# JuliaParallel/DistributedArrays.jl

Measured on NVIDIA H100. Metric: GB/s for map! and sum on Float32 DArray, higher is better.
Workload: dtype f32

## Files before the change

### distributedarrays.jl_b200/_broadcast.py

```python
from __future__ import annotations

import ctypes as C
import struct
from typing import Callable, List, Optional, Sequence, Tuple

import numpy as np

from builtins import any as builtins_any

from . import _lib
from ._darray import B200Array, DArray, dab_dtype, darray, makelocal
from .layout import shape_of
from .runtime import close_remote_reads, open_remote_reads, runtime

_RANK = {"bool": 0, "i32": 1, "i64": 2, "i128": 3, "f32": 4, "f64": 5}


class _TagTypes(dict):

    def __missing__(self, tag):
        raise _lib.UnsupportedError(_lib.ERR_UNSUPPORTED, f"values of type {tag} have no array element type on the GPU backend "
                                    "(Int128 is served as the value type of mapreduce(f, op, d) only)")


# ... 310 lines not shown
        raise _lib.UnsupportedError(_lib.ERR_UNSUPPORTED, "cis of a complex value is not served (complex transcendental functions)")
    e = _float_of(e)
    return Expr("cis", (e,), _CPLX_OF[e.jt])


def complex_(x, y=None) -> Expr:
    e = _traced(x, "complex")
    if y is None:
        if is_ctag(e.jt):
            return e
        if e.jt not in _CPLX_OF:
            raise _lib.UnsupportedError(_lib.ERR_UNSUPPORTED, f"complex({e.jt}) would be Complex{{{e.jt}}}: only ComplexF32 / ComplexF64 are served")
        return convert(e, _CPLX_OF[e.jt])
    f = Expr.wrap(y)
    if is_ctag(e.jt) or is_ctag(f.jt):
        raise TypeError("MethodError: complex(x, y) takes two real parts")
    jt = promote(e.jt, f.jt)
    if jt not in _CPLX_OF:
        raise _lib.UnsupportedError(_lib.ERR_UNSUPPORTED, f"complex of {jt} parts would be Complex{{{jt}}}: only ComplexF32 / ComplexF64 are served")
    return Expr("complex", (convert(e, jt), convert(f, jt)), _CPLX_OF[jt])


def iszero(x) -> Expr:
    return binop("eq", _traced(x, "iszero"), Expr.wrap(0))


def _traced(x, name: str) -> Expr:
    if isinstance(x, Expr):
        return x
    raise TypeError(f"dab.{name} is for use inside broadcast/map kernels")


def uses_complex(e: Expr) -> bool:
    return is_ctag(e.jt) or builtins_any(uses_complex(a) for a in e.args)


def ifelse(c, a, b) -> Expr:
    c, a, b = Expr.wrap(c), Expr.wrap(a), Expr.wrap(b)
    jt = promote(a.jt, b.jt)
    return Expr("ifelse", (convert(c, "bool"), convert(a, jt), convert(b, jt)), jt)


def _mk_unary(name):
    def f(x):
        if isinstance(x, Expr):
            return unop(name, x)
        raise TypeError(f"dab.{name} is for use inside broadcast/map kernels")

    f.__name__ = name
    return f


abs2 = _mk_unary("abs2")
sqrt = _mk_unary("sqrt")
inv = _mk_unary("inv")
floor = _mk_unary("floor")
ceil = _mk_unary("ceil")
sign = _mk_unary("sign")
sin = _mk_unary("sin")
cos = _mk_unary("cos")
tan = _mk_unary("tan")
exp = _mk_unary("exp")
log = _mk_unary("log")
tanh = _mk_unary("tanh")
isnan = _mk_unary("isnan")
isinf = _mk_unary("isinf")
isfinite = _mk_unary("isfinite")
# ... 172 lines not shown
        groups.append((o, ext))
    if not groups:
        groups = [(1, [1] * len(shapes))]
    return tuple(g[0] for g in groups), [tuple(g[1][k] for g in groups) for k in range(len(shapes))]


def _dense_strides(shape):
    s, out = 1, []
    for d in shape:
        out.append(s)
        s *= int(d)
    return out


class LocalArg:

    def __init__(self, arr: Optional[B200Array] = None, scalar=None, tag: str = "f64", temp: bool = False):
        self.arr, self.scalar, self.tag, self.temp = arr, scalar, tag, temp


def run_local(rt, expr: Expr, out: B200Array, largs: List[LocalArg]):
    n = out.size
    if n == 0:
        return
    out_tag = tag_of(out.dtype)
    full = [a for a in largs if a.arr is not None]
    same = all(a.arr.shape == out.shape or a.arr.size == n and _squeeze(a.arr.shape) == _squeeze(out.shape) for a in full)
    ctx = rt.ctx
    code = dab_dtype(out.dtype)
    rt.last_kernel = "fixed"
    cplx = uses_complex(expr) or builtins_any(is_ctag(a.tag) for a in largs)
    if same and not cplx and expr.jt == out_tag and out_tag != "bool":
        x0 = largs[0] if largs and largs[0].arr is not None and largs[0].tag == out_tag else None
        if x0 is not None and all(_only_arg0(expr)):
            ab = match_affine(expr)
            if ab is not None:
                a = np.asarray(ab[0], dtype=out.dtype)
                b = np.asarray(ab[1], dtype=out.dtype)
                _lib.call("dab_affine", ctx, code, C.c_void_p(out.ptr), C.c_void_p(x0.arr.ptr), C.c_void_p(a.ctypes.data),
                          C.c_void_p(b.ctypes.data), n)
                rt.last_kernel = "dab_affine"
                return
            if expr.op in _UN and _is_arg(expr.args[0], 0):
                _lib.call("dab_unary", ctx, code, _UN[expr.op], C.c_void_p(out.ptr), C.c_void_p(x0.arr.ptr), n)
                return
            if _is_arg(expr, 0):
                _lib.call("dab_unary", ctx, code, _lib.MAP_ID, C.c_void_p(out.ptr), C.c_void_p(x0.arr.ptr), n)
                return
        if expr.op in _BIN and len(expr.args) == 2 and not (expr.op == "div" and out_tag[0] != "f"):
            l, r = expr.args
            la = largs[l.val] if l.op == "arg" else None
            ra = largs[r.val] if r.op == "arg" else None

            def arr_ok(e, a):
                return e.op == "arg" and a is not None and a.arr is not None and a.tag == out_tag

            def sc_val(e, a):
                if e.op == "const" and e.jt == out_tag:
                    return e.val
                if e.op == "arg" and a is not None and a.arr is None and a.tag == out_tag:
                    return a.scalar
                return None

            if arr_ok(l, la) and arr_ok(r, ra):
                _lib.call("dab_binary", ctx, code, _BIN[expr.op], C.c_void_p(out.ptr), C.c_void_p(la.arr.ptr), C.c_void_p(ra.arr.ptr), n)
                return
            if arr_ok(l, la) and sc_val(r, ra) is not None:
# ... 43 lines not shown
                    strides[4 * k + d] = 0
                else:
                    raise _lib.DimensionMismatch(_lib.ERR_DIM_MISMATCH, f"arrays could not be broadcast: {a.arr.shape} vs {out.shape}")
        else:
            ptrs[k] = None
            scal[k] = struct.unpack("<Q", np.asarray(a.scalar, dtype=_NPT[a.tag]).tobytes().ljust(8, b"\0"))[0]
    _lib.call("dab_broadcast_expr", ctx, src, code, C.c_void_p(out.ptr), _lib.sz4(oshape), _lib.sz4(_dense_strides(oshape)), nargs, dts,
              ptrs, strides, scal)


def split_c128_scalars(expr: Expr, largs: List["LocalArg"]):
    ks = [k for k, a in enumerate(largs) if a.arr is None and a.tag == "c128"]
    if not ks:
        return expr, largs
    largs, sub = list(largs), {}
    for k in ks:
        z = complex(largs[k].scalar)
        largs[k] = LocalArg(None, z.real, "f64")
        largs.append(LocalArg(None, z.imag, "f64"))
        sub[k] = Expr("complex", (Expr("arg", (), "f64", k), Expr("arg", (), "f64", len(largs) - 1)), "c128")

    def rw(e: Expr) -> Expr:
        if e.op == "arg":
            return sub.get(e.val, e)
        return Expr(e.op, tuple(rw(a) for a in e.args), e.jt, e.val, e.weak) if e.args else e

    return rw(expr), largs


def _squeeze(shape):
    return tuple(s for s in shape if s != 1)


def _only_arg0(e: Expr):
    if e.op == "arg":
        yield e.val == 0
    elif e.op != "const":
        for a in e.args:
            yield from _only_arg0(a)




def _bc_shape(shapes: Sequence[Tuple[int, ...]]) -> Tuple[int, ...]:
    nd = max((len(s) for s in shapes), default=0)
    out = []
    for k in range(nd):
        ext = 1
        for s in shapes:
            v = s[k] if k < len(s) else 1
            if v != 1:
                if ext != 1 and ext != v:
                    raise _lib.DimensionMismatch(_lib.ERR_DIM_MISMATCH, f"arrays could not be broadcast to a common size: {shapes}")
                ext = v
        out.append(ext)
    return tuple(out)


def _arg_tag(a) -> str:
    if isinstance(a, (DArray,)):
        return tag_of(a.dtype)
    if isinstance(a, np.ndarray) and a.ndim > 0:
        return tag_of(a.dtype)
    return Expr.wrap(a.item() if isinstance(a, np.ndarray) else a).jt


def _bcview(arg_dims: Sequence[int], I) -> Tuple:
    out = []
    for k, s in enumerate(arg_dims):
        if s == 1:
            out.append((1, 1))
        elif k < len(I):
# ... 163 lines not shown
```

### distributedarrays.jl_b200/_darray.py

```python
from __future__ import annotations

import ctypes as C
import itertools
import weakref
from typing import Callable, Dict, List, Optional, Sequence, Tuple

import numpy as np

from . import _lib
from .layout import Layout, Range, default_procs, layout_from_chunk_shapes, make_layout, rlen, shape_of, slab_plan
from .runtime import Runtime, close_remote_reads, open_remote_reads, runtime

_DT = {np.dtype(np.float32): _lib.F32, np.dtype(np.float64): _lib.F64, np.dtype(np.int32): _lib.I32,
       np.dtype(np.int64): _lib.I64, np.dtype(np.bool_): _lib.U8,
       np.dtype(np.complex64): _lib.C64, np.dtype(np.complex128): _lib.C128}
_NP = {_lib.F32: np.dtype(np.float32), _lib.F64: np.dtype(np.float64), _lib.I32: np.dtype(np.int32),
       _lib.I64: np.dtype(np.int64), _lib.U8: np.dtype(np.bool_), _lib.C64: np.dtype(np.complex64), _lib.C128: np.dtype(np.complex128)}


def dab_dtype(dt) -> int:
    dt = np.dtype(dt)
    if dt not in _DT:
        raise _lib.UnsupportedError(_lib.ERR_UNSUPPORTED, f"element type {dt} is not served by the GPU backend (no host fallback)")
    return _DT[dt]


def np_dtype(code: int) -> np.dtype:
    return _NP[code]


def is_complex(dt) -> bool:
    return np.dtype(dt).kind == "c"


def component_dtype(dt) -> np.dtype:
    dt = np.dtype(dt)
# ... 2 lines not shown

_allowscalar = [True]


def allowscalar(flag: bool = True):
    _allowscalar[0] = bool(flag)


class B200Array:

    __slots__ = ("rt", "ptr", "shape", "dtype", "_own", "_keep", "_temp")

    def __init__(self, rt: Runtime, ptr: int, shape: Sequence[int], dtype, own: bool = True, keep=None, temp: bool = False):
        self.rt, self.ptr, self.shape, self.dtype = rt, int(ptr), tuple(int(s) for s in shape), np.dtype(dtype)
        self._own, self._keep, self._temp = own, keep, temp

    @classmethod
    def empty(cls, rt: Runtime, shape: Sequence[int], dtype, temp: bool = False) -> "B200Array":
        dtype = np.dtype(dtype)
        n = int(np.prod(shape)) if len(shape) else 1
        ptr = rt.alloc_temp(n * dtype.itemsize) if temp else rt.alloc(n * dtype.itemsize)
        return cls(rt, ptr, shape, dtype, temp=temp)

    @classmethod
    def from_numpy(cls, rt: Runtime, a: np.ndarray) -> "B200Array":
        a = np.asarray(a)
        dab_dtype(a.dtype)
        out = cls.empty(rt, a.shape, a.dtype)
        out.copy_from_host(a)
        return out

    @property
    def size(self) -> int:
        return int(np.prod(self.shape)) if len(self.shape) else 1

    @property
    def nbytes(self) -> int:
        return self.size * self.dtype.itemsize

    @property
    def ndim(self) -> int:
        return len(self.shape)

    def copy_from_host(self, a: np.ndarray, sync: bool = True):
        a = np.asarray(a, dtype=self.dtype)
        if tuple(a.shape) != self.shape:
            raise _lib.DimensionMismatch(_lib.ERR_DIM_MISMATCH, f"host array {a.shape} vs chunk {self.shape}")
        if self.size == 0:
            return
        if not a.flags.f_contiguous:
            if a.ndim == 2 and a.strides[0] == a.itemsize and a.strides[1] > 0:
                _lib.call("dab_h2d_2d", self.rt.ctx, C.c_void_p(self.ptr), a.shape[0] * a.itemsize, C.c_void_p(a.ctypes.data),
                          a.strides[1], a.shape[0] * a.itemsize, a.shape[1])
                if sync:
                    self.rt.sync()
                return
            a = np.asfortranarray(a)
        _lib.call("dab_h2d", self.rt.ctx, C.c_void_p(self.ptr), C.c_void_p(a.ctypes.data), self.nbytes)
        if sync:
            self.rt.sync()

    def to_numpy(self) -> np.ndarray:
        out = np.empty(self.shape, dtype=self.dtype, order="F")
        if self.size:
            _lib.call("dab_d2h", self.rt.ctx, C.c_void_p(out.ctypes.data), C.c_void_p(self.ptr), self.nbytes)
            self.rt.sync()
        return out
# ... 654 lines not shown
```

### distributedarrays.jl_b200/_lib.py

```python
from __future__ import annotations

import ctypes as C
import os

_HERE = os.path.dirname(os.path.abspath(__file__))
SO_PATH = os.path.join(_HERE, "csrc", "libdab200.so")

OK, ERR_CUDA, ERR_ARG, ERR_EMPTY, ERR_DIM_MISMATCH, ERR_NCCL, ERR_UNSUPPORTED, ERR_NVRTC, ERR_NOMEM = range(9)
F32, F64, I32, I64, U8, I128, C64, C128 = range(8)
SUM, PROD, MAX, MIN, ALL, ANY, COUNT, EXTREMA = range(8)
MAP_ID, MAP_ABS, MAP_ABS2, MAP_NEG, MAP_SQRT, MAP_INV, MAP_FLOOR, MAP_CEIL, MAP_SIGN = range(9)
MAP_EQ, MAP_NE, MAP_LT, MAP_LE, MAP_GT, MAP_GE, MAP_ISNAN, MAP_NONZERO = range(16, 24)
FINDMAX, FINDMIN = range(2)
ADD, SUB, MUL, DIV, REM, BMAX, BMIN, MOD, IDIV, AND, OR, XOR = range(12)
SORT_SLICES_SMEM_LEN = 8192
SVDVALS_MAX_K, SVDVALS_MAX_ELEMS = 32, 4096
EIGVALS_SYM_MAX_N = 64
COMPACT_TILE, COMPACT_INDEX = 4096, 0


class DabError(RuntimeError):

    def __init__(self, status: int, msg: str):
        super().__init__(f"[dab status {status}] {msg}")
# ... 73 lines not shown
    "dab_scan_totals": (_i32, [_vp, _i32, _i32, _i32, _vp, _sz, _sz, _sz, _vp]),
    "dab_scan_carrier_dtype": (_i32, [_i32, _i32, _i32, C.POINTER(_i32)]),
    "dab_copy_box": (_i32, [_vp, _i32, _vp, C.POINTER(_sz), C.POINTER(_sz), _vp, C.POINTER(_sz), C.POINTER(_sz), C.POINTER(_sz)]),
    "dab_gather_box": (_i32, [_vp, _i32, _i32, _vp, C.POINTER(C.c_longlong), _pvp, _vp, C.POINTER(C.c_longlong), _pvp, C.POINTER(_sz)]),
    "dab_index_gather": (_i32, [_vp, _i32, _vp, _vp, _i32, _sz, _i32, C.POINTER(_sz), C.POINTER(_i32), C.POINTER(_sz), _pvp, _vp]),
    "dab_compact_count": (_i32, [_vp, _vp, _sz, _sz, _vp]),
    "dab_compact": (_i32, [_vp, _i32, _vp, _vp, _sz, _sz, _vp, _vp, _i32, C.POINTER(_sz), _pvp]),
    "dab_gemv": (_i32, [_vp, _i32, _i32, _vp, _sz, _sz, _vp, _vp]),
    "dab_spmv": (_i32, [_vp, _i32, _sz, _sz, _vp, _vp, _vp, _vp, _vp]),
    "dab_csc_to_csr": (_i32, [_vp, _i32, _sz, _sz, _sz, _vp, _vp, _vp, _vp, _vp, _vp]),
    "dab_gemm": (_i32, [_vp, _i32, _i32, _sz, _sz, _sz, _vp, _sz, _vp, _sz, _vp, _sz]),
    "dab_transpose_box": (_i32, [_vp, _i32, _vp, _sz, _vp, _sz, _sz, _sz]),
    "dab_adjoint_box": (_i32, [_vp, _i32, _vp, _sz, _vp, _sz, _sz, _sz]),
    "dab_sort": (_i32, [_vp, _i32, _vp, _vp, _vp, _sz]),
    "dab_sorted_split": (_i32, [_vp, _i32, _vp, _sz, _vp, _i32, C.POINTER(C.c_ulonglong)]),
    "dab_sort_by_key": (_i32, [_vp, _i32, _vp, _i32, _vp, _vp, _vp, _sz, _sz]),
    "dab_sort_by_key_scratch_bytes": (_i32, [_i32, _sz, C.POINTER(_sz)]),
    "dab_sort_pairs": (_i32, [_vp, _i32, _vp, _vp, _vp, C.c_int64, _vp, _vp, _sz, _sz]),
    "dab_sort_pairs_scratch_bytes": (_i32, [_i32, _sz, C.POINTER(_sz)]),
    "dab_sort_slices": (_i32, [_vp, _i32, _vp, _vp, _sz, _sz, _sz]),
    "dab_svdvals_batched": (_i32, [_vp, _i32, _vp, _sz, _sz, _sz, _vp, _vp]),
    "dab_matmul_batched": (_i32, [_vp, _i32, _sz, _sz, _sz, _vp, _sz, _vp, _sz, _vp, _sz]),
    "dab_eigvals_sym_batched": (_i32, [_vp, _i32, _vp, _sz, _sz, _vp, _vp]),
    "dab_comm_unique_id": (_i32, [_vp]),
    "dab_comm_init_rank": (_i32, [_vp, _vp, _i32, _i32]),
    "dab_comm_destroy": (_i32, [_vp]),
    "dab_allgather": (_i32, [_vp, _vp, _vp, _sz]),
    "dab_allreduce": (_i32, [_vp, _i32, _i32, _vp, _vp, _sz]),
    "dab_group_start": (_i32, [_vp]),
    "dab_group_end": (_i32, [_vp]),
    "dab_send": (_i32, [_vp, _vp, _sz, _i32]),
    "dab_recv": (_i32, [_vp, _vp, _sz, _i32]),
    "dab_mapreduce_all": (_i32, [_vp, _i32, _i32, _i32, _vp, _vp, _sz, _vp]),
    "dab_mailbox_create": (_i32, [_vp, _vp]),
    "dab_mailbox_attach": (_i32, [_vp, _vp, _i32, _i32]),
    "dab_mailbox_detach": (_i32, [_vp]),
    "dab_peer_barrier": (_i32, [_vp]),
    "dab_accumulate_stack": (_i32, [_vp, _i32, _vp, _sz, _vp, _vp, _vp, _sz, _i32]),
    "dab_ipc_get_handle": (_i32, [_vp, _vp, _vp]),
    "dab_ipc_open": (_i32, [_vp, _vp, _pvp]),
    "dab_ipc_close": (_i32, [_vp, _vp]),
    "dab_enable_peer": (_i32, [_vp, _i32]),
}

EXPORTS = tuple(_SIGS)
_NO_STATUS = {"dab_abi_version", "dab_last_error", "dab_status_string"}

_lib = None


def lib() -> C.CDLL:
    global _lib
    if _lib is None:
        if not os.path.exists(SO_PATH):
            raise RuntimeError(
                f"{SO_PATH} is missing: the sm_90a CUDA extension has not been built "
                "(run `python -c 'import __graft_entry__ as g; g.build()'` or `make -C distributedarrays.jl_b200/csrc`). "
                "There is no CPU fallback for the DArray hot path.")
        L = C.CDLL(SO_PATH, mode=C.RTLD_GLOBAL)
        for name, (res, args) in _SIGS.items():
            fn = getattr(L, name)
            fn.restype = res
            fn.argtypes = args
        if L.dab_abi_version() != 1:
            raise RuntimeError("libdab200.so ABI version mismatch")
        _lib = L
# ... 20 lines not shown
```

### distributedarrays.jl_b200/_mapreduce.py

```python
from __future__ import annotations

import builtins
import ctypes as C
import operator
from itertools import accumulate
from typing import Callable, Dict, Optional, Sequence, Tuple

import numpy as np

from . import _lib
from ._broadcast import Expr, broadcast, is_ctag, tag_of, trace, _NPT
from ._darray import B200Array, DArray, component_dtype, dab_dtype, is_complex, np_dtype
from .layout import Layout, ravel, reduction_passes, shape_of, unravel
from .runtime import close_remote_reads, deliver, exchange_stacks, open_remote_reads

_OPS = {"+": _lib.SUM, "add": _lib.SUM, "sum": _lib.SUM, "*": _lib.PROD, "mul": _lib.PROD, "prod": _lib.PROD, "max": _lib.MAX,
        "min": _lib.MIN}
_OPF = {operator.add: _lib.SUM, operator.mul: _lib.PROD, builtins.max: _lib.MAX, builtins.min: _lib.MIN, np.add: _lib.SUM,
        np.multiply: _lib.PROD, np.maximum: _lib.MAX, np.minimum: _lib.MIN}


def _op_code(op) -> int:
    if isinstance(op, str) and op in _OPS:
        return _OPS[op]
    if op in _OPF:
        return _OPF[op]
    raise _lib.UnsupportedError(_lib.ERR_UNSUPPORTED, f"reduction operator {op!r} is not served by a kernel (no host fallback)")


_CMPMAP = {"eq": _lib.MAP_EQ, "ne": _lib.MAP_NE, "lt": _lib.MAP_LT, "le": _lib.MAP_LE, "gt": _lib.MAP_GT, "ge": _lib.MAP_GE}
_FLIP = {"lt": "gt", "le": "ge", "gt": "lt", "ge": "le", "eq": "eq", "ne": "ne"}


def classify_map(f: Optional[Callable], dtype) -> Tuple[Optional[int], Optional[np.ndarray], Optional[Expr]]:
    if f is None:
        return _lib.MAP_ID, None, None
# ... 6 lines not shown
            code = {"abs": _lib.MAP_ABS, "abs2": _lib.MAP_ABS2, "neg": _lib.MAP_NEG, "isnan": _lib.MAP_ISNAN}.get(e.op)
            if code is not None:
                return code, None, e
        return None, None, e
    if e.jt == tag and len(e.args) == 1 and e.args[0].op == "arg":
        code = {"abs": _lib.MAP_ABS, "abs2": _lib.MAP_ABS2, "neg": _lib.MAP_NEG}.get(e.op)
        if code is not None:
            return code, None, e
    if e.op == "mul" and e.jt == tag and builtins.all(a.op == "arg" for a in e.args):
        return _lib.MAP_ABS2, None, e
    if e.op in _CMPMAP:
        l, r = e.args

        def unpromote(side, const):
            if side.op == "convert" and side.args[0].op == "arg" and side.args[0].jt == tag and const.op == "const":
                c = const.val
                if tag == "f32" and const.jt == "f64" and float(np.float32(c)) == c:
                    return side.args[0], Expr("const", (), tag, c)
                if tag in ("i32", "i64") and const.jt in ("i64",) and side.jt == "i64":
                    return side.args[0], Expr("const", (), tag, c) if -2**31 <= c < 2**31 or tag == "i64" else (side, const)
            return side, const

        l, r = unpromote(l, r)
        r, l = unpromote(r, l)
        if l.op == "arg" and r.op == "const" and l.jt == tag:
            return _CMPMAP[e.op], np.asarray(r.val, dtype=np.dtype(dtype)), e
        if r.op == "arg" and l.op == "const" and r.jt == tag:
            return _CMPMAP[_FLIP[e.op]], np.asarray(l.val, dtype=np.dtype(dtype)), e
    if e.op == "isnan" and e.args[0].op == "arg":
        return _lib.MAP_ISNAN, None, e
    return None, None, e


def _result_dtype(dtype, op: int, mapc: int) -> np.dtype:
    out = C.c_int32()
    _lib.check(_lib.lib().dab_reduce_result_dtype(dab_dtype(dtype), op, mapc, C.byref(out)))
    return np.dtype(np.int64) if out.value == _lib.I64 else np_dtype(out.value)




def _gather_slots(d: DArray, launch: Callable[[int, B200Array, int], None]) -> np.ndarray:
    rt = d.rt
    wpr = rt.workers_per_rank
    slots = B200Array.empty(rt, (16 * wpr,), np.uint8, temp=True)
    try:
        for pid, ch in d.chunks.items():
            launch(pid, ch, slots.ptr + 16 * ((pid - 1) % wpr))
        if rt.world > 1:
            allslots = B200Array.empty(rt, (16 * wpr * rt.world,), np.uint8, temp=True)
            _lib.call("dab_allgather", rt.ctx, C.c_void_p(slots.ptr), C.c_void_p(allslots.ptr), 16 * wpr)
            host = allslots.to_numpy()
            allslots.free()
        else:
            host = slots.to_numpy()
    finally:
        rt.sync()
        slots.free()
    return host.view(np.uint8)


def _fold(host: np.ndarray, pids: Sequence[int], rdt: np.dtype, op: int):
    vals = np.empty(len(pids), dtype=rdt)
    for i, pid in enumerate(pids):
        vals[i] = host[16 * (pid - 1):16 * (pid - 1) + rdt.itemsize].view(rdt)[0]
    out = np.zeros(1, dtype=rdt)
# ... 91 lines not shown
        for t in temps:
            t.free()
        close_remote_reads(rt, fenced, "host")
    if wide:
        vals = [_int128(host[16 * (pid - 1):16 * pid].tobytes()) for pid in d.layout.pids]
        res = fold128(vals, opc)
        return (res, vals) if return_partials else res
    res, vals = _fold(host, d.layout.pids, rdt, opc if opc != _lib.COUNT else _lib.SUM)
    return (res, vals) if return_partials else res


def _mapreduce_all(f, op, d: DArray, return_partials: bool = False, others: Sequence = ()):
    opc = op if isinstance(op, int) else _op_code(op)
    if others:
        expr = trace(f, [tag_of(d.dtype)] + [_arg_tag_of(a) for a in others])
        return _mapreduce_expr(expr, opc, d, others, return_partials)
    mapc, param, expr = classify_map(f, d.dtype)
    if is_complex(d.dtype) and mapc is not None and not _complex_served(opc, mapc):
        if mapc == _lib.MAP_ID and opc in (_lib.MAX, _lib.MIN):
            raise TypeError(f"MethodError: no method matching isless(::{d.dtype}, ::{d.dtype}) -- complex numbers are not ordered")
        mapc = None
        if expr is None:
            expr = trace(lambda z: z, [tag_of(d.dtype)])
    if mapc is None:
        return _mapreduce_expr(expr, opc, d, (), return_partials)
    _check_nonempty(d, opc)
    rt = d.rt
    pp = C.c_void_p(param.ctypes.data) if param is not None else None
    rdt = _result_dtype(d.dtype, opc, mapc)
    if rt.workers_per_rank == 1 and d.layout.pids == rt.workers() and not return_partials:
        ch = d.chunks[rt.myid()]
        out = np.zeros(2, dtype=np.uint64)
        _lib.call("dab_mapreduce_all", rt.ctx, dab_dtype(d.dtype), opc, mapc, pp, C.c_void_p(ch.ptr), ch.size, C.c_void_p(out.ctypes.data))
        return out.view(np.uint8)[:rdt.itemsize].view(rdt)[0]
    code = dab_dtype(d.dtype)
    host = _gather_slots(d, lambda pid, ch, slot: _lib.call("dab_reduce", rt.ctx, code, opc, mapc, pp, C.c_void_p(ch.ptr), ch.size, C.c_void_p(slot)))
    res, vals = _fold(host, d.layout.pids, rdt, opc)
    return (res, vals) if return_partials else res


def _complex_served(opc: int, mapc: int) -> bool:
    out = C.c_int32()
    return _lib.lib().dab_reduce_result_dtype(_lib.C64, opc, mapc, C.byref(out)) == _lib.OK


def _arg_tag_of(a) -> str:
    from ._broadcast import _arg_tag
    return _arg_tag(a)


def reduce(op, d: DArray, dims=None, init=None):
    return mapreduce(None, op, d, dims=dims, init=init)


def mapreduce(f: Optional[Callable], op, d: DArray, *ds, dims=None, init=None, _partials: bool = False):
    from ._darray import SubDArray
    if isinstance(d, Expr):
        from . import _slices
        if _slices.tracing():
            return _slices.reduce_of_slice(f, op, d, ds, dims, init)
    if isinstance(d, SubDArray):
        tmp = d.to_darray()
        try:
            return mapreduce(f, op, tmp, *ds, dims=dims, init=init, _partials=_partials)
        finally:
            if dims is None:
                tmp.close()
# ... 383 lines not shown
```

### distributedarrays.jl_b200/csrc/dab_comm.cu

```cuda
#include <dlfcn.h>
#include <nccl.h>

#include "dab_common.cuh"
#include "dab_scalar_ops.cuh"

namespace {

struct NcclApi {
    void* handle = nullptr;
    ncclResult_t (*GetUniqueId)(ncclUniqueId*) = nullptr;
    ncclResult_t (*CommInitRank)(ncclComm_t*, int, ncclUniqueId, int) = nullptr;
    ncclResult_t (*CommDestroy)(ncclComm_t) = nullptr;
    ncclResult_t (*AllGather)(const void*, void*, size_t, ncclDataType_t, ncclComm_t, cudaStream_t) = nullptr;
    ncclResult_t (*AllReduce)(const void*, void*, size_t, ncclDataType_t, ncclRedOp_t, ncclComm_t, cudaStream_t) = nullptr;
    ncclResult_t (*Send)(const void*, size_t, ncclDataType_t, int, ncclComm_t, cudaStream_t) = nullptr;
    ncclResult_t (*Recv)(void*, size_t, ncclDataType_t, int, ncclComm_t, cudaStream_t) = nullptr;
    ncclResult_t (*GroupStart)() = nullptr;
    ncclResult_t (*GroupEnd)() = nullptr;
    const char* (*GetErrorString)(ncclResult_t) = nullptr;
    const char* (*GetLastError)(ncclComm_t) = nullptr;
    bool ok = false;
    char why[256] = "";
};

// ... 159 lines not shown
        default: return dab_fail(ctx, DAB_ERR_ARG, "dab_allreduce: bad op %d", op);
    }
    DAB_NCCL(ctx, api.AllReduce(send_dev, recv_dev, count, dt, ro, (ncclComm_t)ctx->comm, ctx->stream));
    ctx->launches++;
    return DAB_OK;
}

int32_t dab_group_start(dab_ctx* ctx) {
    DAB_ENTER(ctx);
    NEED_COMM(ctx);
    DAB_NCCL(ctx, api.GroupStart());
    return DAB_OK;
}
int32_t dab_group_end(dab_ctx* ctx) {
    DAB_ENTER(ctx);
    NEED_COMM(ctx);
    DAB_NCCL(ctx, api.GroupEnd());
    ctx->launches++;
    return DAB_OK;
}
int32_t dab_send(dab_ctx* ctx, const void* send_dev, size_t nbytes, int32_t peer) {
    DAB_ENTER(ctx);
    NEED_COMM(ctx);
    DAB_NCCL(ctx, api.Send(send_dev, nbytes, ncclInt8, peer, (ncclComm_t)ctx->comm, ctx->stream));
    return DAB_OK;
}
int32_t dab_recv(dab_ctx* ctx, void* recv_dev, size_t nbytes, int32_t peer) {
    DAB_ENTER(ctx);
    NEED_COMM(ctx);
    DAB_NCCL(ctx, api.Recv(recv_dev, nbytes, ncclInt8, peer, (ncclComm_t)ctx->comm, ctx->stream));
    return DAB_OK;
}

int32_t dab_mapreduce_all(dab_ctx* ctx, int32_t dtype, int32_t op, int32_t map, const void* map_param, const void* x, size_t n,
                          void* out_host) {
    DAB_ENTER_NOFLUSH(ctx);
    int32_t rdt;
    if (!out_host || op == DAB_EXTREMA || dab_reduce_result_dtype(dtype, op, map, &rdt) != DAB_OK) {
        DAB_FLUSH(ctx);
        DAB_REQUIRE(ctx, out_host, DAB_ERR_ARG, "dab_mapreduce_all: null out");
        if (op == DAB_EXTREMA) return dab_fail(ctx, DAB_ERR_UNSUPPORTED, "dab_mapreduce_all: extrema combines through dab_reduce + dab_allgather");
        return dab_fail(ctx, DAB_ERR_ARG, "bad dtype/op");
    }
    const bool cplx = rdt == DAB_C64 || rdt == DAB_C128;
    if ((ctx->mbox_ranks > 1 || !ctx->comm || ctx->nranks == 1) && n > 0 && !cplx) {
        ctx->fuse_op = op;
        int32_t st = dab_reduce(ctx, dtype, op, map, map_param, x, n, ctx->result_slot);
        ctx->fuse_op = -1;
        if (st != DAB_OK) return st;
        DAB_CUDA(ctx, cudaStreamSynchronize(ctx->stream));
        const volatile unsigned long long* h = (const volatile unsigned long long*)ctx->host_slot;
        if (h[1] != 0) return dab_fail(ctx, DAB_ERR_NCCL, "fused combine timed out waiting for a peer's chunk result (did every rank call?)");
        unsigned long long bits = h[0];
        memset(out_host, 0, 8);
        memcpy(out_host, &bits, dab_dtype_size(rdt));
        return DAB_OK;
    }
    if (cplx && ctx->mbox_ranks > 1 && !ctx->comm) {
        DAB_FLUSH(ctx);
        return dab_fail(ctx, DAB_ERR_UNSUPPORTED, "dab_mapreduce_all: a complex result across %d ranks needs the NCCL communicator "
                        "(the mailbox combine carries 8-byte results)", ctx->mbox_ranks);
    }
    int32_t st = dab_reduce(ctx, dtype, op, map, map_param, x, n, ctx->result_slot);
    if (st != DAB_OK) return st;
    const int P = ctx->comm ? ctx->nranks : 1;
    const void* src = ctx->result_slot;
    if (P > 1) {
        NEED_COMM(ctx);
        DAB_NCCL(ctx, api.AllGather(ctx->result_slot, ctx->gather_slots, 16, ncclInt8, (ncclComm_t)ctx->comm, ctx->stream));
        ctx->launches++;
        src = ctx->gather_slots;
    }
    DAB_CUDA(ctx, cudaMemcpyAsync(ctx->host_slot, src, (size_t)P * 16, cudaMemcpyDeviceToHost, ctx->stream));
    DAB_CUDA(ctx, cudaStreamSynchronize(ctx->stream));
    unsigned char tmp[DAB_MAX_RANKS * 16];
    size_t es = dab_dtype_size(rdt);
    for (int i = 0; i < P; ++i) memcpy(tmp + (size_t)i * es, (const char*)ctx->host_slot + (size_t)i * 16, es);
    unsigned char res[16] = {0};
    st = dab_combine_ordered(rdt, op, tmp, (size_t)P, res);
    if (st != DAB_OK) return dab_fail(ctx, st, "%s", dab_last_error(nullptr));
    memset(out_host, 0, es > 8 ? es : 8);
    memcpy(out_host, res, es);
    return DAB_OK;
}

int32_t dab_mailbox_create(dab_ctx* ctx, void* handle64) {
    DAB_ENTER(ctx);
    DAB_REQUIRE(ctx, handle64, DAB_ERR_ARG, "dab_mailbox_create: null handle");
// ... 122 lines not shown
```

### distributedarrays.jl_b200/csrc/dab_common.cuh

```cuda
#pragma once
#include <cuda_runtime.h>

#include <cstdint>
#include <cstdio>
#include <cstring>

#include "../../include/dab200.h"

#define DAB_MAX_REDUCE_BLOCKS 262144
#define DAB_SLOT_BYTES 64
#define DAB_MAX_RANKS 64

struct dab_pending_affine {
    int active;
    int32_t dtype;
    void* y;
    const void* x;
    size_t n;
    unsigned char a[8], b[8];
};

struct dab_ctx {
    int device;
    int sm_count;
    cudaStream_t stream;
    void* block_partials;
    unsigned int* counter;
    void* result_slot;
    void* gather_slots;
    void* host_slot;
    void* dim_scratch;
    size_t dim_scratch_bytes;
    uint64_t launches;
    void* comm;
    int rank, nranks;
    void* mailbox;
    void** peer_mbox_dev;
    void* peer_mbox_host[DAB_MAX_RANKS];
    int mbox_ranks;
    unsigned long long mbox_seq;
    unsigned long long barrier_seq;
    int fuse_op;
    struct dab_alloc_cache* cache;
    void* sort_dev;
    size_t sort_dev_bytes;
    void* stage[2];
    cudaEvent_t stage_ev[2];
    void* sort_host;
    unsigned long long sort_epoch;
    void* scan_dev;
    size_t scan_dev_bytes;
    unsigned long long scan_epoch;
    unsigned long long scan_tickets;
    void* scan_scratch;
    size_t scan_scratch_bytes;
    long long opt_combine_timeout_ms;
    int opt_ew_tma;
    dab_pending_affine pending;
    int defer_off;
    char err[512];
};

extern thread_local char dab_tls_err[512];

int32_t dab_fail(dab_ctx* ctx, int32_t status, const char* fmt, ...);
int32_t dab_fail_cuda(dab_ctx* ctx, cudaError_t e, const char* what, const char* file, int line);

#define DAB_CUDA(ctx, call)                                                             \
    do {                                                                                \
        cudaError_t e__ = (call);                                                       \
        if (e__ != cudaSuccess) return dab_fail_cuda((ctx), e__, #call, __FILE__, __LINE__); \
    } while (0)

#define DAB_REQUIRE(ctx, cond, status, ...)                          \
    do {                                                             \
        if (!(cond)) return dab_fail((ctx), (status), __VA_ARGS__);  \
    } while (0)

int32_t dab_flush_pending(dab_ctx* ctx);

#define DAB_FLUSH(ctx)                                    \
    do {                                                  \
        if ((ctx)->pending.active) {                      \
            int32_t st__ = dab_flush_pending(ctx);        \
            if (st__ != DAB_OK) return st__;              \
        }                                                 \
    } while (0)

#define DAB_ENTER(ctx)                                                      \
    do {                                                                    \
// ... 50 lines not shown

template <typename T>
struct alignas(16) Pack {
    static constexpr int N = 16 / sizeof(T);
    T v[N];
};

template <typename T>
struct alignas(2 * sizeof(T)) Cplx {
    T re, im;
};

template <typename T>
__device__ __forceinline__ Pack<T> as_pack(int4 r) {
    Pack<T> p;
    memcpy(&p, &r, 16);
    return p;
}
template <typename T>
__device__ __forceinline__ int4 as_int4(const Pack<T>& p) {
    int4 r;
    memcpy(&r, &p, 16);
    return r;
}

__host__ __device__ __forceinline__ uint32_t dab_hash_u32(uint64_t seed, uint64_t idx) {
    uint64_t z = idx + (seed + 1ull) * 0x9E3779B97F4A7C15ull;
    z = (z ^ (z >> 30)) * 0xBF58476D1CE4E5B9ull;
    z = (z ^ (z >> 27)) * 0x94D049BB133111EBull;
    z = z ^ (z >> 31);
    return (uint32_t)(z >> 32);
}

static inline int dab_grid_for(const dab_ctx* ctx, size_t work_items, int per_sm) {
    size_t cap = (size_t)ctx->sm_count * (size_t)per_sm;
    size_t g = work_items < cap ? work_items : cap;
    return (int)(g < 1 ? 1 : g);
}

int dab_resident_ctas(const void* kernel, int threads);

template <typename K>
static inline int dab_persistent_grid(const dab_ctx* ctx, K kernel, int threads, size_t work_items) {
    return dab_grid_for(ctx, work_items, dab_resident_ctas((const void*)kernel, threads));
}
```

### distributedarrays.jl_b200/csrc/dab_core.cu

```cuda
#include <cstdarg>
#include <cstdlib>
#include <map>
#include <mutex>
#include <new>
#include <thread>
#include <unordered_map>

#include "dab_common.cuh"

thread_local char dab_tls_err[512] = "";

struct dab_alloc_cache {
    std::unordered_map<void*, size_t> live;
    std::multimap<size_t, void*> free_blocks;
    size_t cached_bytes = 0;
    static constexpr size_t kMaxBlock = 16ull << 30;
    static constexpr size_t kMaxCached = 32ull << 30;
};

int dab_resident_ctas(const void* kernel, int threads) {
    static std::mutex mu;
    static std::unordered_map<const void*, int> cache;
    std::lock_guard<std::mutex> lk(mu);
    auto it = cache.find(kernel);
// ... 174 lines not shown
    DAB_ENTER(ctx);
    size_t f = 0, t = 0;
    DAB_CUDA(ctx, cudaMemGetInfo(&f, &t));
    if (device) *device = ctx->device;
    if (sm_count) *sm_count = ctx->sm_count;
    if (free_bytes) *free_bytes = f + (ctx->cache ? ctx->cache->cached_bytes : 0);
    if (total_bytes) *total_bytes = t;
    return DAB_OK;
}

int32_t dab_stream(dab_ctx* ctx, void** stream) {
    DAB_ENTER(ctx);
    DAB_REQUIRE(ctx, stream, DAB_ERR_ARG, "null stream out-pointer");
    ctx->defer_off = 1;
    *stream = (void*)ctx->stream;
    return DAB_OK;
}

int32_t dab_set_option(dab_ctx* ctx, const char* key, int64_t value) {
    if (!ctx || !key) return dab_fail(ctx, DAB_ERR_ARG, "null argument");
    if (ctx->pending.active) {
        DAB_CUDA(ctx, cudaSetDevice(ctx->device));
        DAB_FLUSH(ctx);
    }
    if (strcmp(key, "ew_tma") == 0) {
        ctx->opt_ew_tma = value != 0;
        return DAB_OK;
    }
    if (strcmp(key, "combine_timeout_ms") == 0) {
        if (value < 1) return dab_fail(ctx, DAB_ERR_ARG, "combine_timeout_ms must be >= 1");
        ctx->opt_combine_timeout_ms = value;
        return DAB_OK;
    }
    return dab_fail(ctx, DAB_ERR_ARG, "dab_set_option: unknown key %s", key);
}

int32_t dab_launch_count(dab_ctx* ctx, uint64_t* launches) {
    if (!ctx || !launches) return dab_fail(ctx, DAB_ERR_ARG, "null argument");
    if (ctx->pending.active) {
        DAB_CUDA(ctx, cudaSetDevice(ctx->device));
        DAB_FLUSH(ctx);
    }
    *launches = ctx->launches;
    return DAB_OK;
}

int32_t dab_event_create(dab_ctx* ctx, void** event) {
    DAB_ENTER(ctx);
    DAB_REQUIRE(ctx, event, DAB_ERR_ARG, "null event out-pointer");
    cudaEvent_t ev;
    DAB_CUDA(ctx, cudaEventCreate(&ev));
    *event = (void*)ev;
    return DAB_OK;
}
int32_t dab_event_record(dab_ctx* ctx, void* event) {
    DAB_ENTER(ctx);
    DAB_CUDA(ctx, cudaEventRecord((cudaEvent_t)event, ctx->stream));
    return DAB_OK;
}
int32_t dab_event_elapsed_ms(dab_ctx* ctx, void* start, void* stop, float* ms) {
    DAB_ENTER(ctx);
    DAB_REQUIRE(ctx, ms, DAB_ERR_ARG, "null ms");
    DAB_CUDA(ctx, cudaEventSynchronize((cudaEvent_t)stop));
    DAB_CUDA(ctx, cudaEventElapsedTime(ms, (cudaEvent_t)start, (cudaEvent_t)stop));
    return DAB_OK;
}
// ... 254 lines not shown
```

### distributedarrays.jl_b200/csrc/dab_reduce.cu

```cuda
#include <type_traits>

#include <cmath>

#include "dab_reduce_traits.cuh"

namespace {

struct NoStore {
    template <typename T>
    __device__ __forceinline__ void vec(Pack<T>&, size_t) const {}
    template <typename T>
    __device__ __forceinline__ T scalar(T v, size_t) const { return v; }
};
template <typename T>
struct AffineStore {
    AffineF<T> f;
    T* y;
    int4* yv;
    __device__ __forceinline__ void vec(Pack<T>& p, size_t i) const {
#pragma unroll
        for (int k = 0; k < Pack<T>::N; ++k) p.v[k] = f(p.v[k]);
        st_stream(yv + i, as_int4(p));
    }
    __device__ __forceinline__ T scalar(T v, size_t i) const {
// ... 65 lines not shown
        for (size_t i = ntiles * TILE + threadIdx.x; i < nvec; i += RD_THREADS) {
            Pack<T> p = as_pack<T>(ld_stream(xv + i));
            st.vec(p, i);
            W m = R::pre(map(p.v[0]));
#pragma unroll
            for (int k = 1; k < VPT; ++k) m = R::tile(m, R::pre(map(p.v[k])));
            acc = R::comb(acc, R::lift(m));
        }
        for (size_t i = threadIdx.x; i < head; i += RD_THREADS) acc = R::comb(acc, R::lift(R::pre(map(st.scalar(x[i], i)))));
        for (size_t i = head + nvec * VPT + threadIdx.x; i < n; i += RD_THREADS)
            acc = R::comb(acc, R::lift(R::pre(map(st.scalar(x[i], i)))));
    }
    acc = block_reduce<R>(acc, smem);
    A fin;
    if (!last_cta_out<R>(acc, partials, counter, smem, is_last, fin)) return;
    if (threadIdx.x == 0) {
        if constexpr (std::is_arithmetic<A>::value) {
            Out res;
            if (finalize_mode == 1) res = (Out)(fin == (A)n_for_all);
            else if (finalize_mode == 2) res = (Out)(fin != (A)0);
            else res = (Out)fin;
            memcpy(out, &res, sizeof(Out));
            if (sizeof(Out) < 8) memset((char*)out + sizeof(Out), 0, 8 - sizeof(Out));
            A wide = fin;
            memcpy((char*)out + 8, &wide, sizeof(A));
            if (sizeof(A) < 8) memset((char*)out + 8 + sizeof(A), 0, 8 - sizeof(A));
            if (fc.host_out && fc.nranks <= 1) {
                unsigned long long bits = 0;
                memcpy(&bits, &res, sizeof(Out));
                volatile unsigned long long* h = reinterpret_cast<volatile unsigned long long*>(fc.host_out);
                h[0] = bits;
                h[1] = 0ull;
                __threadfence_system();
            }
        } else if constexpr (is_cplx<Out>::value) {
            using CT = decltype(Out::re);
            const Out res{(CT)fin.re, (CT)fin.im};
            memset(out, 0, 16);
            memcpy(out, &res, sizeof(Out));
        } else {
            memset(out, 0, 16);
            memcpy(out, &fin, sizeof(A));
        }
    }
    if constexpr (!std::is_arithmetic<Out>::value) return;
    else {
    if (fc.nranks <= 1) return;
    __shared__ unsigned long long pay[2];
    __shared__ unsigned long long got[DAB_MAX_RANKS];
    __shared__ int timed_out;
    if (threadIdx.x == 0) {
        memcpy(&pay[0], out, 8);
        memcpy(&pay[1], (char*)out + 8, 8);
        timed_out = 0;
    }
    __syncthreads();
    const size_t bank = (size_t)(fc.seq & 1ull) * DAB_MAX_RANKS * DAB_MBOX_SLOT;
    if (threadIdx.x < (unsigned)fc.nranks) {
        volatile unsigned long long* dst =
            reinterpret_cast<volatile unsigned long long*>((char*)fc.peers[threadIdx.x] + bank + (size_t)fc.rank * DAB_MBOX_SLOT);
        dst[0] = pay[0];
        dst[1] = pay[1];
        __threadfence_system();
        dst[2] = fc.seq;
        volatile unsigned long long* src =
            reinterpret_cast<volatile unsigned long long*>((char*)fc.peers[fc.rank] + bank + (size_t)threadIdx.x * DAB_MBOX_SLOT);
        const unsigned long long t0 = dab_globaltimer_ns();
        unsigned int spins = 0;
        while (src[2] != fc.seq) {
            if ((++spins & 1023u) == 0 && dab_globaltimer_ns() - t0 > fc.timeout_ns) {
                timed_out = 1;
                break;
            }
        }
        __threadfence_system();
        got[threadIdx.x] = src[0];
    }
    __syncthreads();
    if (threadIdx.x == 0) {
        Out a;
        memcpy(&a, &got[0], sizeof(Out));
        for (int j = 1; j < fc.nranks; ++j) {
            Out b;
            memcpy(&b, &got[j], sizeof(Out));
            switch (fc.op) {
                case DAB_SUM: case DAB_COUNT: a = jl::add(a, b); break;
                case DAB_PROD: a = jl::mul(a, b); break;
                case DAB_MAX: a = jl::max(a, b); break;
                case DAB_MIN: a = jl::min(a, b); break;
                case DAB_ALL: a = (Out)(a != (Out)0 && b != (Out)0); break;
                default: a = (Out)(a != (Out)0 || b != (Out)0); break;
            }
        }
        unsigned long long bits = 0;
        memcpy(&bits, &a, sizeof(Out));
        volatile unsigned long long* h = reinterpret_cast<volatile unsigned long long*>(fc.host_out);
        h[0] = bits;
        h[1] = (unsigned long long)timed_out;
        __threadfence_system();
    }
    }
}

template <typename T, typename Map, typename R, typename Out, typename St = NoStore>
int32_t launch_reduce(dab_ctx* ctx, const T* x, size_t n, Map map, void* out, int finalize_mode, St st = St()) {
    const FlatGrid fg = flat_grid(x, n);
    if constexpr (!std::is_same<St, NoStore>::value) st.yv = reinterpret_cast<int4*>(st.y + fg.head);
    FusedComm fc;
    memset(&fc, 0, sizeof(fc));
    if (ctx->fuse_op >= 0 && ctx->mbox_ranks > 1) {
        fc.peers = ctx->peer_mbox_dev;
        fc.host_out = ctx->host_slot;
        fc.seq = ++ctx->mbox_seq;
        fc.timeout_ns = (unsigned long long)ctx->opt_combine_timeout_ms * 1000000ull;
        fc.rank = ctx->rank;
        fc.nranks = ctx->mbox_ranks;
        fc.op = ctx->fuse_op;
    } else if (ctx->fuse_op >= 0) {
        fc.host_out = ctx->host_slot;
        fc.nranks = 1;
        fc.op = ctx->fuse_op;
    }
    reduce_kernel<T, Map, R, Out, St><<<(unsigned)fg.grid, RD_THREADS, 0, ctx->stream>>>(
        x, n, fg.head, map, (typename R::A*)ctx->block_partials, ctx->counter, out, finalize_mode, (long long)n, fg.tiles_per_cta, fc, st);
    DAB_LAUNCHED(ctx);
    return DAB_OK;
}

template <typename T>
using ResultOfSum = typename std::conditional<std::is_floating_point<T>::value, T, long long>::type;

template <typename T, int FN>
int32_t reduce_arith(dab_ctx* ctx, int32_t op, const T* x, size_t n, void* out) {
    MapF<T, FN> map{(T)0};
    switch (op) {
        case DAB_SUM: return launch_reduce<T, MapF<T, FN>, SumTraits<T>, ResultOfSum<T>>(ctx, x, n, map, out, 0);
        case DAB_PROD: return launch_reduce<T, MapF<T, FN>, ProdTraits<T>, ResultOfSum<T>>(ctx, x, n, map, out, 0);
        case DAB_MAX: return launch_reduce<T, MapF<T, FN>, MaxTraits<T>, T>(ctx, x, n, map, out, 0);
        case DAB_MIN: return launch_reduce<T, MapF<T, FN>, MinTraits<T>, T>(ctx, x, n, map, out, 0);
        case DAB_EXTREMA:
            if constexpr (FN == DAB_MAP_ID) return launch_reduce<T, ExtMapF<T>, ExtremaTraits<T>, Pair<T>>(ctx, x, n, ExtMapF<T>{(T)0}, out, 0);
            else return dab_fail(ctx, DAB_ERR_UNSUPPORTED, "extrema with a map is not served (no host fallback)");
        default: return dab_fail(ctx, DAB_ERR_UNSUPPORTED, "reduce op %d needs a predicate map (no host fallback)", op);
    }
}

template <typename T, int FN>
int32_t reduce_pred(dab_ctx* ctx, int32_t op, const T* x, size_t n, const void* param, void* out) {
    PredF<T, FN> map{param ? *(const T*)param : (T)0};
    int mode;
    switch (op) {
        case DAB_ALL: mode = 1; break;
// ... 357 lines not shown
```

### include/dab200.h

```cpp
#ifndef DAB200_H
#define DAB200_H

#include <stddef.h>
#include <stdint.h>

#ifdef __cplusplus
extern "C" {
#endif

#define DAB_ABI_VERSION 1

typedef struct dab_ctx dab_ctx;

enum {
    DAB_OK = 0,
    DAB_ERR_CUDA = 1,
    DAB_ERR_ARG = 2,
    DAB_ERR_EMPTY = 3,
    DAB_ERR_DIM_MISMATCH = 4,
    DAB_ERR_NCCL = 5,
    DAB_ERR_UNSUPPORTED = 6,
    DAB_ERR_NVRTC = 7,
    DAB_ERR_NOMEM = 8
};
// ... 151 lines not shown
int32_t dab_sort_pairs_scratch_bytes(int32_t key_dtype, size_t n, size_t* bytes);
int32_t dab_sort_pairs(dab_ctx* ctx, int32_t key_dtype, const void* keys, void* keys_out, const int64_t* vals, int64_t base,
                       int64_t* vals_out, void* scratch, size_t scratch_bytes, size_t n);

int32_t dab_sorted_split(dab_ctx* ctx, int32_t dtype, const void* sorted, size_t n, const void* bounds_host, int32_t nb,
                         unsigned long long* counts_host);


#define DAB_SORT_SLICES_SMEM_LEN 8192
int32_t dab_sort_slices(dab_ctx* ctx, int32_t dtype, const void* in, void* out, size_t inner, size_t len, size_t outer);

#define DAB_SVDVALS_MAX_K 32
#define DAB_SVDVALS_MAX_ELEMS 4096
int32_t dab_svdvals_batched(dab_ctx* ctx, int32_t dtype, const void* A, size_t m, size_t n, size_t batch, void* S, int32_t* status);


int32_t dab_matmul_batched(dab_ctx* ctx, int32_t dtype, size_t m, size_t n, size_t k, const void* A, size_t strideA, const void* B,
                           size_t strideB, void* C, size_t batch);

#define DAB_EIGVALS_SYM_MAX_N 64
int32_t dab_eigvals_sym_batched(dab_ctx* ctx, int32_t dtype, const void* A, size_t n, size_t batch, void* W, int32_t* status);

int32_t dab_comm_unique_id(void* id128);
int32_t dab_comm_init_rank(dab_ctx* ctx, const void* id128, int32_t rank, int32_t nranks);
int32_t dab_comm_destroy(dab_ctx* ctx);
int32_t dab_allgather(dab_ctx* ctx, const void* send_dev, void* recv_dev, size_t nbytes_per_rank);
int32_t dab_allreduce(dab_ctx* ctx, int32_t dtype, int32_t op, const void* send_dev, void* recv_dev, size_t count);
int32_t dab_group_start(dab_ctx* ctx);
int32_t dab_group_end(dab_ctx* ctx);
int32_t dab_send(dab_ctx* ctx, const void* send_dev, size_t nbytes, int32_t peer);
int32_t dab_recv(dab_ctx* ctx, void* recv_dev, size_t nbytes, int32_t peer);
int32_t dab_mapreduce_all(dab_ctx* ctx, int32_t dtype, int32_t op, int32_t map, const void* map_param, const void* x,
                          size_t n, void* out_host);

int32_t dab_mailbox_create(dab_ctx* ctx, void* handle64);
int32_t dab_mailbox_attach(dab_ctx* ctx, const void* handles, int32_t rank, int32_t nranks);
int32_t dab_mailbox_detach(dab_ctx* ctx);

int32_t dab_peer_barrier(dab_ctx* ctx);
int32_t dab_accumulate_stack(dab_ctx* ctx, int32_t dtype, void* y, size_t n, const void* beta, const void* alpha, const void* stack,
                             size_t stride, int32_t count);

int32_t dab_ipc_get_handle(dab_ctx* ctx, const void* dptr, void* handle64);
int32_t dab_ipc_open(dab_ctx* ctx, const void* handle64, void** dptr);
int32_t dab_ipc_close(dab_ctx* ctx, void* dptr);
int32_t dab_enable_peer(dab_ctx* ctx, int32_t peer_device);

#ifdef __cplusplus
}
#endif
#endif
```

Before: 4243.

## Poll a sequence-tagged host result word instead of synchronizing the stream in mapreduce_all

The fused reduce kernel now writes a sequence number after its result into the pinned host slot. The host spins on that word with a deadline instead of calling cudaStreamSynchronize, so the result is returned as soon as it lands rather than after stream-completion signalling. The change also removes Python-side overhead: non-generator _only_arg0 and uses_complex, math.prod for size, a cached result dtype, and a simpler result view. It adds optional host timing instrumentation. The trade-offs are busy-wait CPU use, extra stream queries, and reliance on correct memory ordering of the host-visible writes.

After: 4312, median of 6. No clear change (+1.6%).

```diff
diff --git a/distributedarrays.jl_b200/_broadcast.py b/distributedarrays.jl_b200/_broadcast.py
--- a/distributedarrays.jl_b200/_broadcast.py
+++ b/distributedarrays.jl_b200/_broadcast.py
@@ -366,7 +366,12 @@
 
 
 def uses_complex(e: Expr) -> bool:
-    return is_ctag(e.jt) or builtins_any(uses_complex(a) for a in e.args)
+    if e.jt in _COMP:
+        return True
+    for a in e.args:
+        if uses_complex(a):
+            return True
+    return False
 
 
 def ifelse(c, a, b) -> Expr:
@@ -605,7 +610,7 @@
     cplx = uses_complex(expr) or builtins_any(is_ctag(a.tag) for a in largs)
     if same and not cplx and expr.jt == out_tag and out_tag != "bool":
         x0 = largs[0] if largs and largs[0].arr is not None and largs[0].tag == out_tag else None
-        if x0 is not None and all(_only_arg0(expr)):
+        if x0 is not None and _only_arg0(expr):
             ab = match_affine(expr)
             if ab is not None:
                 a = np.asarray(ab[0], dtype=out.dtype)
@@ -715,12 +720,14 @@
     return tuple(s for s in shape if s != 1)
 
 
-def _only_arg0(e: Expr):
+def _only_arg0(e: Expr) -> bool:
     if e.op == "arg":
-        yield e.val == 0
-    elif e.op != "const":
+        return e.val == 0
+    if e.op != "const":
         for a in e.args:
-            yield from _only_arg0(a)
+            if not _only_arg0(a):
+                return False
+    return True
 
 
 
diff --git a/distributedarrays.jl_b200/_darray.py b/distributedarrays.jl_b200/_darray.py
--- a/distributedarrays.jl_b200/_darray.py
+++ b/distributedarrays.jl_b200/_darray.py
@@ -2,6 +2,7 @@
 
 import ctypes as C
 import itertools
+import math
 import weakref
 from typing import Callable, Dict, List, Optional, Sequence, Tuple
 
@@ -70,7 +71,7 @@
 
     @property
     def size(self) -> int:
-        return int(np.prod(self.shape)) if len(self.shape) else 1
+        return math.prod(self.shape)
 
     @property
     def nbytes(self) -> int:
diff --git a/distributedarrays.jl_b200/_lib.py b/distributedarrays.jl_b200/_lib.py
--- a/distributedarrays.jl_b200/_lib.py
+++ b/distributedarrays.jl_b200/_lib.py
@@ -129,6 +129,8 @@
     "dab_send": (_i32, [_vp, _vp, _sz, _i32]),
     "dab_recv": (_i32, [_vp, _vp, _sz, _i32]),
     "dab_mapreduce_all": (_i32, [_vp, _i32, _i32, _i32, _vp, _vp, _sz, _vp]),
+    "dab_wait_word": (_i32, [_vp, C.c_ulonglong, C.c_ulonglong, _vp]),
+    "dab_host_timing": (_i32, [_vp, C.POINTER(_u64)]),
     "dab_mailbox_create": (_i32, [_vp, _vp]),
     "dab_mailbox_attach": (_i32, [_vp, _vp, _i32, _i32]),
     "dab_mailbox_detach": (_i32, [_vp]),
diff --git a/distributedarrays.jl_b200/_mapreduce.py b/distributedarrays.jl_b200/_mapreduce.py
--- a/distributedarrays.jl_b200/_mapreduce.py
+++ b/distributedarrays.jl_b200/_mapreduce.py
@@ -2,6 +2,7 @@
 
 import builtins
 import ctypes as C
+import functools
 import operator
 from itertools import accumulate
 from typing import Callable, Dict, Optional, Sequence, Tuple
@@ -74,6 +75,7 @@
     return None, None, e
 
 
+@functools.lru_cache(maxsize=None)
 def _result_dtype(dtype, op: int, mapc: int) -> np.dtype:
     out = C.c_int32()
     _lib.check(_lib.lib().dab_reduce_result_dtype(dab_dtype(dtype), op, mapc, C.byref(out)))
@@ -231,7 +233,7 @@
         ch = d.chunks[rt.myid()]
         out = np.zeros(2, dtype=np.uint64)
         _lib.call("dab_mapreduce_all", rt.ctx, dab_dtype(d.dtype), opc, mapc, pp, C.c_void_p(ch.ptr), ch.size, C.c_void_p(out.ctypes.data))
-        return out.view(np.uint8)[:rdt.itemsize].view(rdt)[0]
+        return out.view(rdt)[0]
     code = dab_dtype(d.dtype)
     host = _gather_slots(d, lambda pid, ch, slot: _lib.call("dab_reduce", rt.ctx, code, opc, mapc, pp, C.c_void_p(ch.ptr), ch.size, C.c_void_p(slot)))
     res, vals = _fold(host, d.layout.pids, rdt, opc)
diff --git a/distributedarrays.jl_b200/csrc/dab_comm.cu b/distributedarrays.jl_b200/csrc/dab_comm.cu
--- a/distributedarrays.jl_b200/csrc/dab_comm.cu
+++ b/distributedarrays.jl_b200/csrc/dab_comm.cu
@@ -215,6 +215,29 @@
     return DAB_OK;
 }
 
+int32_t dab_wait_word(const void* slot, unsigned long long seq, unsigned long long deadline_ns, void* out16) {
+    const unsigned long long* w = (const unsigned long long*)slot;
+    for (unsigned int spins = 0;; ++spins) {
+        if (__atomic_load_n(w + 2, __ATOMIC_ACQUIRE) == seq) {
+            const unsigned long long v[2] = {__atomic_load_n(w, __ATOMIC_RELAXED), __atomic_load_n(w + 1, __ATOMIC_RELAXED)};
+            memcpy(out16, v, 16);
+            return 1;
+        }
+        if ((spins & 63u) == 0 && dab_host_ns() >= deadline_ns) return 0;
+#if defined(__x86_64__)
+        __builtin_ia32_pause();
+#elif defined(__aarch64__)
+        asm volatile("yield");
+#endif
+    }
+}
+
+int32_t dab_host_timing(dab_ctx* ctx, uint64_t* out3) {
+    if (!ctx || !out3) return dab_fail(ctx, DAB_ERR_ARG, "null argument");
+    memcpy(out3, ctx->host_t, sizeof(ctx->host_t));
+    return DAB_OK;
+}
+
 int32_t dab_mapreduce_all(dab_ctx* ctx, int32_t dtype, int32_t op, int32_t map, const void* map_param, const void* x, size_t n,
                           void* out_host) {
     DAB_ENTER_NOFLUSH(ctx);
@@ -227,16 +250,36 @@
     }
     const bool cplx = rdt == DAB_C64 || rdt == DAB_C128;
     if ((ctx->mbox_ranks > 1 || !ctx->comm || ctx->nranks == 1) && n > 0 && !cplx) {
+        if (ctx->opt_host_timing) ctx->host_t[0] = dab_host_ns();
+        volatile unsigned long long* h = (volatile unsigned long long*)ctx->host_slot;
+        h[2] = 0;
         ctx->fuse_op = op;
         int32_t st = dab_reduce(ctx, dtype, op, map, map_param, x, n, ctx->result_slot);
         ctx->fuse_op = -1;
         if (st != DAB_OK) return st;
-        DAB_CUDA(ctx, cudaStreamSynchronize(ctx->stream));
-        const volatile unsigned long long* h = (const volatile unsigned long long*)ctx->host_slot;
-        if (h[1] != 0) return dab_fail(ctx, DAB_ERR_NCCL, "fused combine timed out waiting for a peer's chunk result (did every rank call?)");
-        unsigned long long bits = h[0];
+        if (ctx->opt_host_timing) ctx->host_t[1] = dab_host_ns();
+        const unsigned long long seq = ctx->mbox_seq;
+        const unsigned long long deadline = dab_host_ns() + (unsigned long long)ctx->opt_combine_timeout_ms * 1000000ull;
+        unsigned long long res[2];
+        for (;;) {
+            const unsigned long long now = dab_host_ns();
+            if (dab_wait_word(ctx->host_slot, seq, now + 1000000ull < deadline ? now + 1000000ull : deadline, res)) break;
+            const cudaError_t q = cudaStreamQuery(ctx->stream);
+            if (q == cudaErrorNotReady) (void)cudaGetLastError();
+            else if (q != cudaSuccess) return dab_fail_cuda(ctx, q, "cudaStreamQuery", __FILE__, __LINE__);
+            if (q == cudaSuccess || dab_host_ns() >= deadline) {
+                DAB_CUDA(ctx, cudaStreamSynchronize(ctx->stream));
+                if (dab_wait_word(ctx->host_slot, seq, 0, res)) break;
+                return dab_fail(ctx, DAB_ERR_CUDA, "dab_mapreduce_all: the reduce kernel finished without writing its result word");
+            }
+        }
+        const cudaError_t q = cudaStreamQuery(ctx->stream);
+        if (q == cudaErrorNotReady) (void)cudaGetLastError();
+        else if (q != cudaSuccess) return dab_fail_cuda(ctx, q, "cudaStreamQuery", __FILE__, __LINE__);
+        if (ctx->opt_host_timing) ctx->host_t[2] = dab_host_ns();
+        if (res[1] != 0) return dab_fail(ctx, DAB_ERR_NCCL, "fused combine timed out waiting for a peer's chunk result (did every rank call?)");
         memset(out_host, 0, 8);
-        memcpy(out_host, &bits, dab_dtype_size(rdt));
+        memcpy(out_host, &res[0], dab_dtype_size(rdt));
         return DAB_OK;
     }
     if (cplx && ctx->mbox_ranks > 1 && !ctx->comm) {
diff --git a/distributedarrays.jl_b200/csrc/dab_common.cuh b/distributedarrays.jl_b200/csrc/dab_common.cuh
--- a/distributedarrays.jl_b200/csrc/dab_common.cuh
+++ b/distributedarrays.jl_b200/csrc/dab_common.cuh
@@ -4,6 +4,7 @@
 #include <cstdint>
 #include <cstdio>
 #include <cstring>
+#include <ctime>
 
 #include "../../include/dab200.h"
 
@@ -56,6 +57,8 @@
     size_t scan_scratch_bytes;
     long long opt_combine_timeout_ms;
     int opt_ew_tma;
+    int opt_host_timing;
+    unsigned long long host_t[3];
     dab_pending_affine pending;
     int defer_off;
     char err[512];
@@ -172,6 +175,12 @@
     return (uint32_t)(z >> 32);
 }
 
+static inline unsigned long long dab_host_ns() {
+    timespec ts;
+    clock_gettime(CLOCK_MONOTONIC, &ts);
+    return (unsigned long long)ts.tv_sec * 1000000000ull + (unsigned long long)ts.tv_nsec;
+}
+
 static inline int dab_grid_for(const dab_ctx* ctx, size_t work_items, int per_sm) {
     size_t cap = (size_t)ctx->sm_count * (size_t)per_sm;
     size_t g = work_items < cap ? work_items : cap;
diff --git a/distributedarrays.jl_b200/csrc/dab_core.cu b/distributedarrays.jl_b200/csrc/dab_core.cu
--- a/distributedarrays.jl_b200/csrc/dab_core.cu
+++ b/distributedarrays.jl_b200/csrc/dab_core.cu
@@ -230,6 +230,11 @@
         ctx->opt_combine_timeout_ms = value;
         return DAB_OK;
     }
+    if (strcmp(key, "host_timing") == 0) {
+        ctx->opt_host_timing = value != 0;
+        memset(ctx->host_t, 0, sizeof(ctx->host_t));
+        return DAB_OK;
+    }
     return dab_fail(ctx, DAB_ERR_ARG, "dab_set_option: unknown key %s", key);
 }
 
diff --git a/distributedarrays.jl_b200/csrc/dab_reduce.cu b/distributedarrays.jl_b200/csrc/dab_reduce.cu
--- a/distributedarrays.jl_b200/csrc/dab_reduce.cu
+++ b/distributedarrays.jl_b200/csrc/dab_reduce.cu
@@ -121,6 +121,7 @@
                 h[0] = bits;
                 h[1] = 0ull;
                 __threadfence_system();
+                h[2] = fc.seq;
             }
         } else if constexpr (is_cplx<Out>::value) {
             using CT = decltype(Out::re);
@@ -187,6 +188,7 @@
         h[0] = bits;
         h[1] = (unsigned long long)timed_out;
         __threadfence_system();
+        h[2] = fc.seq;
     }
     }
 }
@@ -207,6 +209,7 @@
         fc.op = ctx->fuse_op;
     } else if (ctx->fuse_op >= 0) {
         fc.host_out = ctx->host_slot;
+        fc.seq = ++ctx->mbox_seq;
         fc.nranks = 1;
         fc.op = ctx->fuse_op;
     }
diff --git a/include/dab200.h b/include/dab200.h
--- a/include/dab200.h
+++ b/include/dab200.h
@@ -207,6 +207,8 @@
 int32_t dab_recv(dab_ctx* ctx, void* recv_dev, size_t nbytes, int32_t peer);
 int32_t dab_mapreduce_all(dab_ctx* ctx, int32_t dtype, int32_t op, int32_t map, const void* map_param, const void* x,
                           size_t n, void* out_host);
+int32_t dab_wait_word(const void* slot, unsigned long long seq, unsigned long long deadline_ns, void* out16);
+int32_t dab_host_timing(dab_ctx* ctx, uint64_t* out3);
 
 int32_t dab_mailbox_create(dab_ctx* ctx, void* handle64);
 int32_t dab_mailbox_attach(dab_ctx* ctx, const void* handles, int32_t rank, int32_t nranks);
```
